# TheMTank/GridUniverse

Measured on AMD Instinct MI355X. Metric: env-steps/sec at N_envs on 32×32 grid, 1/2/4/8 MI355X; bit-exact vs CPU, higher is better.
Workload: dtype int32; 1 GPU; c3: 65536 envs per GPU on the 32x32 generator maze (random.seed(123); np.random.seed(123)), uniform device-RNG actions, auto-reset, 1000 env-steps per launch, int32 (obs,reward,done) rows; envs_per_gpu=65536, env_steps_per_launch=1000, global_envs=65536, parallelism=env-index shards, no data-path collective

## Files before the change

### griduniverse_amd/csrc/gu_internal.hpp

```cpp
#pragma once
#include <hip/hip_runtime.h>
#include <stdint.h>
#include <atomic>
#include <string>
#include <vector>

#include "../../include/gu.h"
#include "../../include/gu_diag.h"

#define GU_CELL_OPEN_MASK 0x0Fu
#define GU_CELL_TERM 0x10u
#define GU_CELL_TERM_BIT 4
#define GU_CELL_RPLUS 0x20u
#define GU_CELL_RMINUS 0x40u
#define GU_WIDE_STORE_PAD()                         \
    do {                                            \
        __builtin_amdgcn_sched_barrier(0);          \
        asm volatile("s_nop 1" ::: "memory");       \
        __builtin_amdgcn_sched_barrier(0);          \
    } while (0)
#define GU_ACTION_OK(raw) ((uint32_t)((int32_t)(raw) + 4) < 8u)
#define GU_CELL_WALL 0x80u

#define GU_MAX_LDS_CELLS 32767

#define GU_HOST_ERR_WORD 4
#define GU_HOST_COUNT_WORD 8

#define GU_STREAM_PAD_WORDS 4

struct GuPaceEntry {
    uint32_t period_q;
    uint32_t seq;
    uint64_t t_start;
    uint32_t unpaced;
    uint32_t phase;
    uint32_t left;
    uint32_t ema_paced;
    uint32_t ema_unpaced;
    uint32_t verdict;
    uint32_t waves;
    uint32_t elapsed;
    uint32_t ended_late;
    uint32_t max_behind;
    uint32_t report_steps;
    uint32_t groups;
    uint32_t dec_q;
    uint32_t block_left;
    uint32_t block_sum;
    uint32_t block_n;
    uint32_t last_mean;
    uint32_t up;
    uint32_t quiet;
    uint32_t reserved2[9];
};
static_assert(sizeof(GuPaceEntry) == 128, "GuPaceEntry is two cache lines' halves: 128 bytes");
#define GU_PACE_BLOCK 192u
#define GU_PACE_BLOCK_SKIP 64u
#define GU_PACE_NORMAL 0
#define GU_PACE_PROBE_OFF 1
#define GU_PACE_OFF 2
#define GU_PACE_PROBE_ON 3
#define GU_PACE_RING 64u
struct GuPaceArgs {
    GuPaceEntry *ring;
    uint64_t *slots;
    uint32_t seq;
    uint32_t period;
    uint32_t lo, hi;
    uint32_t groups;
    uint32_t report_at;
    uint32_t n_waves, slot_stride;
    uint16_t bar_num;
    uint16_t fixed;
    uint32_t gain_q;
    uint32_t dec_q;
    uint32_t probe_every;
    uint32_t adapt;
};

struct gu_engine {
    int device = -1;
    int n_cu = 256;
    int64_t lds_per_cu = 160 * 1024;
    bool gfx950 = true;
    int64_t opt[GU_OPT_COUNT];
    int64_t opt_x[GU_OPT_X_COUNT];
    hipStream_t stream = nullptr;
    hipEvent_t ev_begin = nullptr, ev_end = nullptr, ev_sync = nullptr;
    std::vector<hipEvent_t> ev_marks;
    size_t n_marks = 0;

    int64_t N = 0;
    int64_t env_id0 = 0;

    bool has_grid = false;
    int32_t W = 0, H = 0, S = 0;
    int32_t cell_bytes = 0;
    uint8_t *d_cell = nullptr;
    uint8_t *d_cell_raw = nullptr;
    uint8_t *d_kind = nullptr;
    uint64_t delta_lut = 0;
    int32_t *d_starts = nullptr;
    int32_t *d_nstarts = nullptr;
    int32_t n_starts = 0;
    int32_t start0 = 0;
    int32_t max_starts = 0;
    bool all_single_start = true;
    int32_t n_grids = 1;
    int64_t group = 0;

    int32_t *d_out3 = nullptr;
    uint32_t *d_episode = nullptr;
    int32_t *d_out3_alt = nullptr;
    uint32_t *d_episode_alt = nullptr;
    uint64_t *d_done_bits_alt = nullptr;
    uint32_t *d_nib = nullptr;
    bool nib_valid = false;
    uint32_t *d_tcount = nullptr;
    uint64_t steps_taken = 0;
    int64_t off_lo = 0, off_hi = 0;
    bool off_exact = true;
    uint64_t seed = 0;
    uint32_t seed_prefix = 0;

    int32_t *d_actions = nullptr;
    uint32_t *d_actions_packed = nullptr;
    int64_t actions_T = 0;
    int64_t actions_cap = 0;

    int32_t *d_traj = nullptr;
    int64_t traj_T = 0;
    int traj_kind = 0;
    int traj_written = 0;
    int32_t traj_candidates = 0;
    float traj_probe_ms_best = 0.0f, traj_probe_ms_worst = 0.0f;
    std::vector<float> traj_probe_ms;
    std::vector<uint64_t> traj_probe_addr;
    int32_t traj_kept = -1;
    float traj_search_ms = 0.0f;
    uint64_t traj_peak_bytes = 0;
    bool traj_registered = false;

    struct PaceKind {
        bool active = false;
        const void *buffer = nullptr;
        unsigned blocks = 0;
        int64_t T = 0;
        int row_bytes = 0;
        uint32_t seq = 0;
        uint32_t model = 0;
        uint32_t n_waves = 0;
    } pace[36];
    GuPaceEntry *d_pace_ring = nullptr;
    uint64_t *d_pace_slots = nullptr;
    int64_t pace_slot_stride = 0;
    hipEvent_t ev_cal[2] = {nullptr, nullptr};

    uint32_t *d_rows[2] = {nullptr, nullptr};
    int rows_shift[2] = {-1, -1};
    uint32_t *d_rows2[2] = {nullptr, nullptr};
    bool rows2_built[2] = {false, false};
    uint32_t *d_mrows[2] = {nullptr, nullptr}, *d_mrows1[2] = {nullptr, nullptr};
    int mrows_K[2] = {0, 0}, mrows_shift[2] = {-1, -1};
    uint32_t *d_prow = nullptr;

    int32_t *d_ret = nullptr;
    int32_t *d_episodes_fin = nullptr;
    bool stats_valid = false;

    uint64_t *d_done_bits = nullptr;
    bool entry_table_ok = false;
    bool done_bits_valid = false;

    void *d_scratch = nullptr;
    size_t scratch_bytes = 0;

    int32_t *h_pin = nullptr;
    double *h_tables = nullptr;
    size_t h_tables_bytes = 0;
    bool h_tables_valid = false;
    unsigned long long *h_ctl = nullptr;
    char *h_up = nullptr;
    uint32_t *h_seq = nullptr;
    uint32_t *d_blocks_done = nullptr;
    uint32_t seq = 0, seq_since_sync = 0;

    hipGraphExec_t graph_exec = nullptr;
    int64_t graph_t0 = -1, graph_T = -1;
    uint32_t graph_flags = 0;

    double *d_v[2] = {nullptr, nullptr};
    double *d_pi[2] = {nullptr, nullptr};
    uint4 *d_pi_thr = nullptr;
    int vi_cur = 0;
    bool has_vi = false;
    double *d_delta = nullptr;
    uint8_t *d_greedy = nullptr;
    bool greedy_valid = false;
    int32_t vi_xcd_members[8] = {0, 0, 0, 0, 0, 0, 0, 0};
    int vi_run_form = 0;
    void *d_vi_xcd_ctl = nullptr, *d_vi_xcd_work = nullptr;
    size_t vi_xcd_ctl_bytes = 0, vi_xcd_work_bytes = 0;
    uint32_t vi_xcd_epoch = 1;
    int64_t vi_xcd_torn = 0;
    int vi_dp_form = 0;

    double *d_q = nullptr;
    int8_t *d_td_next = nullptr;
    int32_t td_S = 0;
    bool td_carry = false;
    int32_t *d_nstep_sa = nullptr;
    int32_t *d_nstep_r = nullptr;
    int32_t *d_nstep_cnt = nullptr;
    int32_t nstep_key = 0;
    int32_t *d_lambda_w = nullptr;
    int32_t lambda_key = 0;
    double *d_ac_h = nullptr;
    double *d_ac_v = nullptr;
    int32_t ac_S = 0;
    int32_t *d_rf_buf = nullptr;
    int32_t *d_rf_cnt = nullptr;
    int32_t rf_cap = 0;
    int32_t rf_key = 0;
    double *d_is_c = nullptr;
    int32_t is_S = 0;
    double *d_is_R = nullptr;
    int64_t is_eps = -1;
    int32_t *d_is_buf = nullptr;
    int32_t *d_is_cnt = nullptr;
    int32_t is_cap = 0;
    int32_t is_key = 0;
    double *d_fa_w = nullptr;
    int32_t *d_fa_phi = nullptr;
    uint16_t *d_fa_phi16 = nullptr;
    size_t fa_phi16_bytes = 0;
    int8_t *d_fa_next = nullptr;
    int32_t fa_S = 0, fa_K = 0, fa_F = 0;
    bool fa_carry = false;
    uint64_t *d_dyna_model = nullptr;
    int32_t *d_dyna_list = nullptr;
    int32_t *d_dyna_count = nullptr;
    uint8_t *d_dyna_seen = nullptr;
    int32_t dyna_S = 0;
    bool dyna_exact = false;
    double *d_search_score = nullptr;
    int64_t *d_search_steps = nullptr;
    uint32_t *d_explore_n = nullptr;
    int32_t explore_S = 0;
    double *d_explore_tab = nullptr;
    int32_t explore_C = 0;
    uint8_t *d_mcts_pool = nullptr;
    int32_t *d_mcts_meta = nullptr;
    int32_t *d_mcts_nodes = nullptr;
    int64_t *d_mcts_steps = nullptr;
    int32_t mcts_P = 0;
    double *d_mcts_tab = nullptr;
    int32_t mcts_C = 0;

    int32_t trail_cap = 0;
    int32_t *d_trail = nullptr;
    int32_t *d_trail_len = nullptr, *d_trail_head = nullptr;
    uint8_t *d_trail_done = nullptr;
    uint32_t *d_trail_alpha = nullptr;

    void *comm = nullptr;
    int32_t nranks = 0, rank = 0;
    int32_t *d_gather = nullptr;

    int32_t *pos() const { return d_out3; }
    int32_t *reward() const { return d_out3 + N; }
    int32_t *done() const { return d_out3 + 2 * N; }
};

struct GridSel {
    int64_t group;
    int64_t grid_stride;
    const int32_t *n_starts;
    int32_t n_grids, max_starts;
    int32_t per_wave;
};

inline GridSel gu_grid_sel(const gu_engine *h)
{
    return GridSel{h->group, 2 * (int64_t)h->cell_bytes, h->d_nstarts, h->n_grids, h->max_starts, 0};
}

void gu_set_error(const char *fmt, ...);
int gu_fail(int code, const char *fmt, ...);

#define GU_HIP(expr)                                                                              \
    do {                                                                                          \
        hipError_t _e = (expr);                                                                   \
        if (_e != hipSuccess)                                                                     \
            return gu_fail(_e == hipErrorOutOfMemory ? GU_ERR_NOMEM : GU_ERR_HIP, "%s failed: %s", \
                           #expr, hipGetErrorString(_e));                                         \
    } while (0)

#define GU_REQUIRE(cond, code, ...) \
    do {                            \
        if (!(cond)) return gu_fail(code, __VA_ARGS__); \
    } while (0)

int gu_use_device(gu_engine *h);
int gu_ensure_scratch(gu_engine *h, size_t bytes);

#define GU_TRY(call)                                 \
    do {                                             \
        int _rc = (call);                            \
        if (_rc != GU_OK) return _rc;                \
    } while (0)

#define GU_ENTER(h) GU_TRY(gu_use_device(h))

#define GU_NEED_GRID(h) GU_REQUIRE((h)->has_grid, GU_ERR_STATE, "no grid set: call gu_set_grid first")

template <class... P>
static inline void gu_release(P *&...p)
{
    ((p ? (void)hipFree(p) : (void)0, p = nullptr), ...);
}

int64_t gu_opt(const gu_engine *h, int option);
int gu_debug();

template <typename K>
static inline void gu_allow_lds(K kern, std::atomic<uint64_t> &mask, int device, size_t bytes, size_t wanted)
{
    if (bytes <= 64 * 1024) return;
    const uint64_t bit = device < 64 ? (1ull << device) : 0;
    if (bit && (mask.load(std::memory_order_relaxed) & bit)) return;
    (void)hipFuncSetAttribute((const void *)kern, hipFuncAttributeMaxDynamicSharedMemorySize, (int)wanted);
    if (bit) mask.fetch_or(bit, std::memory_order_relaxed);
}

int gu_launch_reset(gu_engine *h, const uint8_t *d_mask, const int32_t *d_choice, bool only_done);
int gu_launch_step(gu_engine *h, const int32_t *d_actions_row, uint32_t flags, int32_t *host_obs = nullptr,
                   int32_t *host_reward = nullptr, int32_t *host_done = nullptr, uint32_t *host_seq = nullptr, uint32_t seq = 0,
                   uint32_t *host_err = nullptr);
int gu_launch_validate_actions(gu_engine *h, const int32_t *d_actions, int64_t count);
int gu_launch_pack_actions(gu_engine *h, int64_t T);
int gu_launch_rollout(gu_engine *h, int64_t T, int32_t policy, uint32_t flags);
int gu_launch_lookahead(gu_engine *h, int64_t n, const int32_t *d_states, const int32_t *d_actions, bool care,
                        int32_t *d_next, int32_t *d_reward, int32_t *d_done);
int gu_launch_done_compact(gu_engine *h);
int gu_launch_deinterleave(gu_engine *h, const int32_t *triples, int32_t *planes, int64_t count);
int gu_probe_trajectory_buffer(gu_engine *h, int32_t *buf, int64_t T, float *ms);
int gu_device_copy(gu_engine *h, void *dst, const void *src, size_t bytes);
#define GU_MAX_SEGMENTS 8
struct GuSegments {
    void *dst[GU_MAX_SEGMENTS];
    const void *src[GU_MAX_SEGMENTS];
    size_t words[GU_MAX_SEGMENTS];
    int n = 0;
    void add(void *d, const void *s, size_t bytes)
    {
        dst[n] = d, src[n] = s, words[n] = bytes / 4;
        ++n;
    }
};
int gu_device_segments(gu_engine *h, const GuSegments &s);
#define GU_CTL_WORDS (8 + 4096 + 20480)
#define GU_UP_BYTES (40 * 4096)
int gu_read_back(gu_engine *h, void *dst, const void *src, size_t bytes);

int gu_vi_alloc(gu_engine *h);
void gu_vi_free(gu_engine *h);
int gu_launch_greedy_table(gu_engine *h);

struct GuXcdPlan {
    int block = 0, K = 0, NB = 1;
    unsigned G = 0;
    uint32_t values = 0;
    size_t lds = 0, slots_bytes = 0, work_bytes = 0;
};
#define GU_VI_FALLBACK 1
bool gu_vi_xcd_plan(const gu_engine *h, bool agents, GuXcdPlan *plan);
void gu_vi_xcd_free(gu_engine *h);
int gu_vi_xcd_fused_run(gu_engine *h, const GuXcdPlan &xp, double gamma, int32_t iters, uint32_t flags, double *deltas);
int gu_vi_xcd_dp_run(gu_engine *h, double gamma, double threshold, bool use_threshold, bool greedy, int32_t max_rounds, int32_t *rounds_done,
                     double *deltas);

// ... 34 lines not shown
```

### griduniverse_amd/csrc/gu_rollout.hpp

```cpp
#pragma once
#include "gu_map.hpp"

#include <cstdlib>
#include <functional>
#include <type_traits>

__device__ __forceinline__ uint32_t gu_sample_action(uint32_t word, const uint4 q)
{
    return (uint32_t)(word >= q.x) + (uint32_t)(word >= q.y) + (uint32_t)(word >= q.z) - q.w;
}


#define GU_DPP_REDUCE(x, OP)                                                                                     \
    do {                                                                                                         \
        uint32_t o_;                                                                                             \
        o_ = (uint32_t)__builtin_amdgcn_update_dpp(0, (int)(x), 0x111, 0xF, 0xF, false), (x) = OP((x), o_);      \
        o_ = (uint32_t)__builtin_amdgcn_update_dpp(0, (int)(x), 0x112, 0xF, 0xF, false), (x) = OP((x), o_);      \
        o_ = (uint32_t)__builtin_amdgcn_update_dpp(0, (int)(x), 0x114, 0xF, 0xF, false), (x) = OP((x), o_);      \
        o_ = (uint32_t)__builtin_amdgcn_update_dpp(0, (int)(x), 0x118, 0xF, 0xF, false), (x) = OP((x), o_);      \
        o_ = (uint32_t)__builtin_amdgcn_update_dpp(0, (int)(x), 0x142, 0xA, 0xF, false), (x) = OP((x), o_);      \
        o_ = (uint32_t)__builtin_amdgcn_update_dpp(0, (int)(x), 0x143, 0xC, 0xF, false), (x) = OP((x), o_);      \
    } while (0)
#define GU_OP_ADD(a_, b_) ((a_) + (b_))
#define GU_OP_MAX(a_, b_) ((a_) > (b_) ? (a_) : (b_))

struct GuPacer {
    uint64_t due, t0;
    uint32_t ticks;
    uint32_t report_at;
    uint32_t n_steps;
    uint32_t p_q;
    uint64_t *slot;
    uint64_t w[16];
    uint32_t c_seq, c_phase, c_left, c_ema_p, c_ema_u, v_period_q, v_seq, v_unpaced, v_report_steps, v_groups;
    uint32_t c_dec_q, c_block_left, c_block_sum, c_block_n, c_last_mean, c_up, c_quiet;
    uint64_t v_t_start;
    bool first_wave;
    __device__ __forceinline__ void fetch(const GuPaceArgs &pa, bool on)
    {
        ticks = on ? pa.period : 0u;
        p_q = pa.period << 6;
        first_wave = false;
        if (on && pa.ring) {
            const GuPaceEntry *entry = pa.ring + (pa.seq & (GU_PACE_RING - 1u));
            const GuPaceEntry *prev = pa.ring + ((pa.seq - 1u) & (GU_PACE_RING - 1u));
            c_seq = entry->seq;
            const bool mine = c_seq == pa.seq;
            const uint32_t have = mine ? entry->period_q : 0u;
            const uint32_t unpaced = mine ? entry->unpaced : 0u;
            c_phase = entry->phase, c_left = entry->left, c_ema_p = entry->ema_paced, c_ema_u = entry->ema_unpaced;
            v_period_q = prev->period_q, v_seq = prev->seq, v_unpaced = prev->unpaced, v_t_start = prev->t_start;
            v_report_steps = prev->report_steps, v_groups = prev->groups;
            if (have && !pa.fixed) p_q = have;
            p_q = p_q < (pa.lo << 6) ? (pa.lo << 6) : p_q;
            p_q = p_q > (pa.hi << 6) ? (pa.hi << 6) : p_q;
            if (pa.fixed) p_q = pa.period << 6;
            ticks = (unpaced && !pa.fixed) ? 0u : (p_q + 32u) >> 6;
            c_quiet = (mine && !pa.fixed) ? entry->quiet : 0u;
            first_wave = blockIdx.x == 0 && __builtin_amdgcn_readfirstlane(threadIdx.x) < 64u;
            if (first_wave && !c_quiet) {
                c_dec_q = entry->dec_q, c_block_left = entry->block_left, c_block_sum = entry->block_sum, c_block_n = entry->block_n;
                c_last_mean = entry->last_mean, c_up = entry->up;
                const uint64_t *set = pa.slots + (size_t)((pa.seq - 1u) & 1u) * pa.slot_stride;
#pragma unroll
                for (uint32_t j = 0; j < 16u; ++j) {
                    const uint32_t i = j * 64u + threadIdx.x;
                    w[j] = i < pa.n_waves ? __builtin_nontemporal_load(set + i) : 0ull;
                }
            }
        }
    }
    __device__ __forceinline__ void start(const GuPaceArgs &pa, bool on)
    {
        slot = nullptr;
        n_steps = 0;
        report_at = 0;
        t0 = 0;
        if (on && pa.ring) {
            const uint64_t now = __builtin_amdgcn_s_memrealtime();
            due = t0 = now;
            if (c_quiet) {
                if (first_wave) decide_quiet(pa, now);
                return;
            }
            const uint32_t wave = __builtin_amdgcn_readfirstlane((blockIdx.x * blockDim.x + threadIdx.x) >> 6);
            slot = pa.slots + (size_t)(pa.seq & 1u) * pa.slot_stride + wave;
            report_at = pa.report_at;
            if (first_wave) decide(pa, now);
            return;
        }
        due = ticks ? __builtin_amdgcn_s_memrealtime() : 0ull;
    }
    __device__ __forceinline__ void decide_early(const GuPaceArgs &pa)
    {
        if (first_wave && !c_quiet) decide(pa, __builtin_amdgcn_s_memrealtime());
    }
    __device__ __forceinline__ void decide_quiet(const GuPaceArgs &pa, uint64_t now)
    {
        first_wave = false;
        if (threadIdx.x == 0) {
            GuPaceEntry *cur = pa.ring + (pa.seq & (GU_PACE_RING - 1u));
            GuPaceEntry *next = pa.ring + ((pa.seq + 1u) & (GU_PACE_RING - 1u));
            uint32_t ema_u = c_ema_u;
            const uint64_t gap = now - v_t_start;
            const uint32_t took = gap > 0x7FFFFFFFull ? 0x7FFFFFFFu : (uint32_t)gap;
            if (v_seq + 1u == pa.seq && v_unpaced && v_t_start && v_groups == pa.groups && (!ema_u || took < 2u * ema_u)) ema_u = ema_u ? (ema_u * 7u + took) >> 3 : took;
            cur->t_start = now, cur->groups = pa.groups, cur->report_steps = 0;
            const uint32_t left = c_left > 0u ? c_left - 1u : 0u;
            next->period_q = p_q, next->seq = pa.seq + 1u, next->t_start = 0, next->unpaced = 1u;
            next->phase = GU_PACE_OFF, next->left = left, next->ema_paced = c_ema_p, next->ema_unpaced = ema_u;
            next->verdict = 0, next->waves = 0, next->elapsed = 0, next->ended_late = 0, next->max_behind = 0, next->report_steps = 0, next->groups = 0;
            next->dec_q = pa.dec_q, next->block_left = GU_PACE_BLOCK, next->block_sum = 0, next->block_n = 0, next->last_mean = 0, next->up = 0;
            next->quiet = left > 1u ? 1u : 0u;
        }
    }
    __device__ __forceinline__ void decide(const GuPaceArgs &pa, uint64_t now)
    {
        first_wave = false;
        uint64_t *set = pa.slots + (size_t)((pa.seq - 1u) & 1u) * pa.slot_stride;
        GuPaceEntry *cur = pa.ring + (pa.seq & (GU_PACE_RING - 1u));
        GuPaceEntry *prev = pa.ring + ((pa.seq - 1u) & (GU_PACE_RING - 1u));
        const bool fresh = c_seq != pa.seq;
        const bool prev_ok = v_seq + 1u == pa.seq;
        const uint32_t prev_ticks = (prev_ok && !v_unpaced) ? (pa.fixed ? pa.period : (v_period_q + 32u) >> 6) : 0u;
        const uint32_t scheduled = (prev_ticks * ((v_report_steps + 15u) & ~15u)) >> 4;
        const bool same_length = v_groups == pa.groups;
        uint32_t counts = 0, most = 0, longest = 0;
        for (uint32_t base = 0; base < pa.n_waves; base += 64u * 16u) {
            if (base) {
#pragma unroll
                for (uint32_t j = 0; j < 16u; ++j) {
                    const uint32_t i = base + j * 64u + threadIdx.x;
                    w[j] = i < pa.n_waves ? __builtin_nontemporal_load(set + i) : 0ull;
                }
            }
#pragma unroll
            for (uint32_t j = 0; j < 16u; ++j) {
                const uint32_t i = base + j * 64u + threadIdx.x;
                if (i < pa.n_waves) set[i] = 0;
                const uint32_t reported = (uint32_t)(w[j] >> 63), elapsed = (uint32_t)w[j] & 0x7FFFFFFFu;
                const uint32_t behind = (prev_ticks && elapsed > scheduled) ? elapsed - scheduled : 0u;
                counts += (reported << 16) + ((reported && behind > 2u * prev_ticks) ? 1u : 0u);
                most = behind > most ? behind : most;
                longest = elapsed > longest ? elapsed : longest;
            }
        }
        GU_DPP_REDUCE(counts, GU_OP_ADD);
        GU_DPP_REDUCE(most, GU_OP_MAX);
        GU_DPP_REDUCE(longest, GU_OP_MAX);
        if (threadIdx.x == 63) {
            const uint32_t waves = counts >> 16, far = counts & 0xFFFFu;
            GuPaceEntry *next = pa.ring + ((pa.seq + 1u) & (GU_PACE_RING - 1u));
            uint32_t n_q = p_q, phase = GU_PACE_NORMAL, left = pa.probe_every ? (pa.probe_every < 128u ? pa.probe_every : 128u) : 0u, ema_p = 0, ema_u = 0;
            uint32_t dec_q = pa.dec_q, block_left = GU_PACE_BLOCK, block_sum = 0, block_n = 0, last_mean = 0, up = 0;
            if (!fresh) {
                phase = c_phase, left = c_left, ema_p = c_ema_p, ema_u = c_ema_u;
                dec_q = c_dec_q, block_left = c_block_left, block_sum = c_block_sum, block_n = c_block_n, last_mean = c_last_mean, up = c_up;
            } else {
                cur->unpaced = 0, cur->phase = phase, cur->left = left, cur->ema_paced = 0, cur->ema_unpaced = 0;
                cur->dec_q = dec_q, cur->block_left = block_left, cur->block_sum = 0, cur->block_n = 0, cur->last_mean = 0, cur->up = up;
            }
            cur->period_q = p_q, cur->seq = pa.seq, cur->t_start = now, cur->report_steps = pa.report_at, cur->groups = pa.groups;
            cur->verdict = 0, cur->waves = 0, cur->elapsed = 0, cur->ended_late = 0, cur->max_behind = 0;
            if (waves && prev_ok) {
                prev->verdict = (uint64_t)most * 256u > (uint64_t)prev_ticks * v_groups * pa.bar_num ? 2u : 1u;
                prev->waves = waves, prev->elapsed = longest, prev->ended_late = far, prev->max_behind = far ? most : 0u;
                const uint64_t gap = now - v_t_start;
                const uint32_t mean = v_unpaced ? ema_u : ema_p;
                const uint32_t took = gap > 0x7FFFFFFFull ? 0x7FFFFFFFu : (uint32_t)gap;
                const bool plausible = same_length && v_t_start && (!mean || took < 2u * mean);
                if (v_unpaced) {
                    if (plausible) ema_u = ema_u ? (ema_u + took) >> 1 : took;
                } else {
                    if (plausible) ema_p = ema_p ? (ema_p * 7u + took) >> 3 : took;
                    const uint32_t step_up = (uint32_t)(((uint64_t)pa.gain_q * far) / waves);
                    const uint32_t early = 512u / (8u + (pa.seq > 100000u ? 100000u : pa.seq));
                    const uint32_t dec = early > dec_q ? early : dec_q;
                    n_q += step_up;
                    n_q = n_q > dec ? n_q - dec : n_q;
                    if (phase == GU_PACE_NORMAL && !pa.fixed && pa.adapt) {
                        if (block_left <= GU_PACE_BLOCK - GU_PACE_BLOCK_SKIP && plausible) block_sum += took, ++block_n;
                        if (block_left) --block_left;
                        if (!block_left) {
                            const uint32_t mean = block_n ? block_sum / block_n : 0u;
                            if (mean && last_mean && mean > last_mean) up ^= 1u;
                            if (mean) last_mean = mean;
                            dec_q = up ? (dec_q * 4u + 2u) / 3u : (dec_q * 3u) / 4u;
                            dec_q = dec_q < 4u ? 4u : dec_q;
                            dec_q = dec_q > pa.gain_q / 8u ? pa.gain_q / 8u : dec_q;
                            block_left = GU_PACE_BLOCK, block_sum = 0, block_n = 0;
                        }
                    }
                }
            }
            n_q = n_q < (pa.lo << 6) ? (pa.lo << 6) : n_q;
            n_q = n_q > (pa.hi << 6) ? (pa.hi << 6) : n_q;
            if (pa.probe_every && !pa.fixed && left && --left == 0u) {
                const bool off_wins = ema_u && ema_p && (uint64_t)ema_u * 100u < (uint64_t)ema_p * 98u;
                if (phase != GU_PACE_NORMAL || off_wins) block_left = GU_PACE_BLOCK, block_sum = 0, block_n = 0, last_mean = 0;
                if (phase == GU_PACE_NORMAL) phase = GU_PACE_PROBE_OFF, left = 4u, ema_u = 0u;
                else if (phase == GU_PACE_OFF) phase = GU_PACE_PROBE_ON, left = 8u, ema_p = 0u;
                else if (off_wins) phase = GU_PACE_OFF, left = 2u * pa.probe_every;
                else phase = GU_PACE_NORMAL, left = pa.probe_every;
            }
            next->period_q = n_q, next->seq = pa.seq + 1u, next->t_start = 0;
            next->unpaced = (phase == GU_PACE_PROBE_OFF || phase == GU_PACE_OFF) ? 1u : 0u;
            next->phase = phase, next->left = left, next->ema_paced = ema_p, next->ema_unpaced = ema_u;
            next->dec_q = dec_q, next->block_left = block_left, next->block_sum = block_sum, next->block_n = block_n, next->last_mean = last_mean, next->up = up;
            next->quiet = (phase == GU_PACE_OFF && left > 1u) ? 1u : 0u;
            next->verdict = 0, next->waves = 0, next->elapsed = 0, next->ended_late = 0, next->max_behind = 0, next->report_steps = 0, next->groups = 0;
        }
    }
    __device__ __forceinline__ void report(uint64_t now)
    {
        if ((threadIdx.x & 63u) == 0u) {
            const uint64_t elapsed = now - t0;
            *slot = (1ull << 63) | (elapsed > 0x7FFFFFFFull ? 0x7FFFFFFFull : elapsed);
        }
        report_at = 0;
    }
    __device__ __forceinline__ bool idle() const { return ticks == 0u && slot == nullptr; }
    __device__ __forceinline__ void after(uint32_t steps)
    {
        if (ticks) {
            due += (ticks * steps) >> 4;
            const uint64_t now = __builtin_amdgcn_s_memrealtime();
            n_steps += steps;
            if (__builtin_expect(report_at != 0u && n_steps >= report_at, 0)) report(now);
            if ((int64_t)(now - due) < 0)
                for (uint32_t turn = 0; turn < 2u * ticks + 64u && (int64_t)(__builtin_amdgcn_s_memrealtime() - due) < 0; ++turn)
                    __builtin_amdgcn_s_sleep(1);
        } else if (slot) {
            n_steps += steps;
            if (__builtin_expect(report_at != 0u && n_steps >= report_at, 0)) report(__builtin_amdgcn_s_memrealtime());
        }
    }
    __device__ __forceinline__ void finish()
    {
        if (slot && report_at) report(__builtin_amdgcn_s_memrealtime());
    }
};

struct RolloutArgs {
    const uint8_t *cell;
    const uint8_t *greedy;
    const uint4 *pi_thr;
    int32_t S, pi_lds;
    int32_t cell_bytes, W;
    uint64_t lut;
    int32_t *pos, *reward, *done;
    uint32_t *episode;
    const uint32_t *tcount;
    const int32_t *starts;
    const uint32_t *actions;
    int32_t *tr_obs, *tr_reward, *tr_done;
    int32_t *ret, *episodes_fin;
    uint64_t *done_bits;
    uint32_t n_starts, seed_prefix, env_id0, steps_taken;
    uint32_t seed_prefix0, steps_hi;
    const uint32_t *nib;
    int32_t nib_dwords;
    uint64_t lut_p;
    int32_t straddle;
    int64_t N, T;
    GridSel gs;
    const uint32_t *rows;
    const uint32_t *rows2;
    int32_t row_shift;
    int32_t stream_lds_off;
    int32_t stream_lds_words;
    int32_t entry_table;
    int32_t half_waves;
    int32_t xcd_remap;
    GuPaceArgs pace;
};

__device__ __forceinline__ uint32_t gu_env_block(int32_t xcd_remap)
{
    const uint32_t b = blockIdx.x;
    return xcd_remap ? (b & 7u) * (gridDim.x >> 3) + (b >> 3) : b;
}

template <bool TAIL16 = false, class S16, class S1>
__device__ __forceinline__ void gu_stream_run(const char *pa, int64_t row, uint32_t e4, int64_t T, int64_t i0, S16 &&step16, S1 &&step1)
{
    const uint32_t row32 = (uint32_t)row;
    auto word_at = [&](int64_t k, uint32_t c) {
        return (uint32_t)__builtin_amdgcn_raw_buffer_load_b32(__builtin_amdgcn_make_buffer_rsrc((void *)(pa + k * row), 0, 0xFFFFFFFFu, 0x00020000), e4,
                                                              c * row32, 0);
    };
    int64_t i = i0, k = i0 >> 4;
    if (i & 15) {
        const uint32_t word = word_at(k, 0);
        for (; i < T && (i & 15); ++i) step1((word >> (2u * (uint32_t)(i & 15))) & 3u);
        ++k;
    }
    uint32_t w[4];
#pragma unroll
    for (uint32_t c = 0; c < 4; ++c) w[c] = word_at(k, c);
    for (const int64_t full = T >> 4; k + 4 <= full; k += 4, i += 64) {
#pragma unroll
        for (uint32_t c = 0; c < 4; ++c) {
            const uint32_t word = w[c];
            asm volatile("" ::"v"(word));
            w[c] = word_at(k + 4, c);
            step16(word);
        }
    }
    uint32_t q = 0;
    if (TAIL16) {
        for (; i + 16 <= T; i += 16, q += 16) {
            const uint32_t sel = q >> 4;
            step16(sel == 0 ? w[0] : sel == 1 ? w[1] : w[2]);
        }
    }
    for (; i < T; ++i, ++q) {
        const uint32_t sel = q >> 4, word = sel == 0 ? w[0] : sel == 1 ? w[1] : sel == 2 ? w[2] : w[3];
        step1((word >> (2u * (q & 15u))) & 3u);
    }
}

#ifndef GU_STORE_AUX
#define GU_STORE_AUX 18
#endif
#ifndef GU_STORE_AUX_PACKED
#define GU_STORE_AUX_PACKED 16
#endif
#define GU_MAX_BLOCK 1024
typedef uint32_t gu_v3u __attribute__((ext_vector_type(3)));
template <int POLICY, int AUTO, int TRAJ, bool STATS, int MAP>
__global__ void __launch_bounds__(GU_MAX_BLOCK) gu_rollout_kernel(const RolloutArgs a)
{
    constexpr bool LDS = MAP == 1 || MAP == 3;
    extern __shared__ __attribute__((aligned(16))) uint8_t smem[];
    GuPacer pacer;
    pacer.fetch(a.pace, TRAJ == 1 || TRAJ == 3);
    const int64_t e64 = (int64_t)gu_env_block(a.xcd_remap) * blockDim.x + threadIdx.x;
    const bool live = e64 < a.N;
    const uint32_t e = (uint32_t)e64;
    int32_t s = 0, r = 0;
    uint32_t d = 0, ep = 0, tcount0 = 0;
    if (live) {
        s = a.pos[e];
        r = a.reward[e];
        d = (uint32_t)a.done[e];
        ep = a.episode[e];
        tcount0 = a.tcount[e];
    }
    CellMap m = gu_stage_map<LDS>(a.cell, a.cell_bytes, smem, a.gs, MAP == 3 ? 1 : 2);
    const uint32_t nib_region = MAP == 5 ? (threadIdx.x >> 6) * (uint32_t)a.nib_dwords * 256u : 0u;
    if (MAP == 5) {
        const size_t wave = ((size_t)blockIdx.x * blockDim.x + threadIdx.x) >> 6;
        const uint4 *src = reinterpret_cast<const uint4 *>(a.nib + wave * (size_t)a.nib_dwords * 64u);
        uint4 *dst = reinterpret_cast<uint4 *>(smem + nib_region);
        if (wave * 64u < (size_t)a.N)
            for (int32_t i = threadIdx.x & 63; i < a.nib_dwords * 16; i += 64) dst[i] = src[i];
        __syncthreads();
    }
    const uint8_t *greedy = a.greedy;
    if (MAP == 1 && POLICY == GU_POLICY_GREEDY) {
        uint8_t *dst = smem + 2 * a.cell_bytes;
        for (int32_t i = threadIdx.x * 16; i < a.cell_bytes; i += blockDim.x * 16)
            *reinterpret_cast<uint4 *>(dst + i) = *reinterpret_cast<const uint4 *>(a.greedy + i);
        __syncthreads();
        greedy = dst;
    }
    const bool thr_in_lds = MAP == 1 && POLICY == GU_POLICY_SAMPLE && a.pi_lds;
    uint4 *thr_lds = reinterpret_cast<uint4 *>(smem + 2 * a.cell_bytes);
    if (thr_in_lds) {
        for (int32_t i = threadIdx.x; i < a.S; i += blockDim.x) thr_lds[i] = a.pi_thr[i];
        __syncthreads();
    }
    if (!live) return;
    LaneGrid lg = gu_lane_grid<LDS>(a.gs, a.starts, a.n_starts, e, m);

    const uint32_t t_lane = tcount0 + a.steps_taken;
    const uint32_t prefix = gu_rng_prefix(a.seed_prefix, a.env_id0 + e);
    const uint32_t prefix0 = AUTO == 2 ? gu_rng_prefix(a.seed_prefix0, a.env_id0 + e) : prefix;
    const uint32_t epoch0 = (uint32_t)((uint64_t)((int64_t)(((uint64_t)a.steps_hi << 32) | a.steps_taken) + (int64_t)(int32_t)tcount0) >> 32);
    auto prefix_at = [&](uint32_t t) {
        return gu_rng_prefix(gu_rng_seed_prefix_epoch(a.seed_prefix0, epoch0 + (t < t_lane ? 1u : 0u)), a.env_id0 + e);
    };
    constexpr uint32_t TERM5 = 0x20u, TERM5_BIT = 5u;
    auto flags5 = [](uint32_t b) { return (((b >> 5) & 3u) << 3) | (((b >> GU_CELL_TERM_BIT) & 1u) << TERM5_BIT) | ((b >> 7) << 6); };
    uint32_t flags = MAP == 5 ? flags5(m.f[s]) : m.f[s];
    int32_t ret = 0, fin = 0;
    const int32_t W = a.W;
    const uint64_t lut = a.lut;
    const int32_t start0 = lg.starts[0];
    const uint32_t start0_flags = MAP == 5 ? flags5(m.f[start0]) : m.f[start0];
    auto padded = [&](int32_t c) { return (int32_t)(((uint32_t)(c + c / W + W + 2) << 5) + nib_region); };
    int32_t sq = MAP == 5 ? padded(s) : 0;
    const int32_t start0_q = MAP == 5 ? padded(start0) : 0;
    typedef __attribute__((address_space(3))) const uint32_t *lds_word_ptr;
    const uint32_t lane4 = (threadIdx.x & 63u) << 2;
    auto word_at = [&](int32_t cq) { return *(lds_word_ptr)(uintptr_t)(((uint32_t)cq & 0xFFFFFF00u) | lane4); };
    auto four_of = [](uint32_t word, int32_t cq) { return __builtin_amdgcn_ubfe(word, (uint32_t)cq >> 3, 4); };
    auto four_at = [&](int32_t cq) { return four_of(word_at(cq), cq); };
    auto cell5 = [&](int32_t cq) { return four_at(cq) << 3; };
    auto move5 = [&](uint32_t act, int32_t delta, auto &&in_the_shadow) {
        int32_t cand = s + delta;
        asm volatile("" : "+v"(cand));
        const int32_t candq = sq + gu_delta<true>(act, a.lut_p, 0);
        const uint32_t word = word_at(candq);
        in_the_shadow();
        const uint32_t four = four_of(word, candq);
        const bool go = ((flags & TERM5) | four) < 8u;
        s = go ? cand : s;
        sq = go ? candq : sq;
        flags = go ? four << 3 : flags;
    };
    char *po = (char *)a.tr_obs, *pr = (char *)a.tr_reward, *pd = (char *)a.tr_done;
    const char *pa = (const char *)a.actions;
    const uint32_t e4 = e * 4u;
    const int64_t row = a.N * 4;
    const uint32_t row32 = (uint32_t)row;
    const int64_t trow = TRAJ == 3 ? a.N * 12 : row;
    const uint32_t trow32 = (uint32_t)trow;
    const uint32_t te = TRAJ == 3 ? e * 12u : e4;
    __amdgpu_buffer_rsrc_t ro = __builtin_amdgcn_make_buffer_rsrc(po, 0, 0xFFFFFFFFu, 0x00020000);
    __amdgpu_buffer_rsrc_t rr = __builtin_amdgcn_make_buffer_rsrc(pr, 0, 0xFFFFFFFFu, 0x00020000);
    __amdgpu_buffer_rsrc_t rd = __builtin_amdgcn_make_buffer_rsrc(pd, 0, 0xFFFFFFFFu, 0x00020000);
    auto emit = [&](int32_t s_, int32_t r_, uint32_t d_, uint32_t soff) {
        if (TRAJ == 1) {
            __builtin_amdgcn_raw_buffer_store_b32(s_, ro, e4, soff, GU_STORE_AUX);
            __builtin_amdgcn_raw_buffer_store_b32(r_, rr, e4, soff, GU_STORE_AUX);
            __builtin_amdgcn_raw_buffer_store_b32((int32_t)d_, rd, e4, soff, GU_STORE_AUX);
        } else if (TRAJ == 2) {
            __builtin_amdgcn_raw_buffer_store_b32((int32_t)((uint32_t)s_ | (((uint32_t)r_ & 0xFFu) << 16) | (d_ << 24)), ro, e4, soff, GU_STORE_AUX_PACKED);
        } else if (TRAJ == 3) {
            const gu_v3u triple = {(uint32_t)s_, (uint32_t)r_, d_};
            __builtin_amdgcn_raw_buffer_store_b96(triple, ro, te, soff, GU_STORE_AUX);
            GU_WIDE_STORE_PAD();
        }
    };
    bool held = false;
    int32_t held_s = 0, held_r = 0;
    uint32_t held_d = 0, held_soff = 0;
    auto release = [&]() {
        if (MAP == 5 && TRAJ && held) emit(held_s, held_r, held_d, held_soff);
        held = false;
    };
    auto rebase = [&](int64_t rows) {
        release();
        po += rows * trow;
        ro = __builtin_amdgcn_make_buffer_rsrc(po, 0, 0xFFFFFFFFu, 0x00020000);
        if (TRAJ == 1) {
            pr += rows * trow;
            pd += rows * trow;
            rr = __builtin_amdgcn_make_buffer_rsrc(pr, 0, 0xFFFFFFFFu, 0x00020000);
            rd = __builtin_amdgcn_make_buffer_rsrc(pd, 0, 0xFFFFFFFFu, 0x00020000);
        }
    };

    if (AUTO == 1 && MAP != 5) flags = (flags & ~GU_CELL_TERM) | (d << GU_CELL_TERM_BIT);

    auto step = [&](uint32_t act, uint32_t soff) {
        const int32_t delta = gu_delta<MAP != 0>(act, lut, W);
        if (AUTO == 1) {
            const bool was_done = MAP == 5 ? d != 0u : (flags & GU_CELL_TERM) != 0u;
            ep += was_done;
            s = was_done ? start0 : s;
            flags = was_done ? start0_flags : flags;
            if (MAP == 5) sq = was_done ? start0_q : sq;
        } else if (AUTO == 2) {
            if (d) {
                s = lg.starts[gu_rng_start_index(prefix0, ep, lg.n_starts)];
                ++ep;
                if (MAP == 5) sq = padded(s);
                flags = MAP == 5 ? cell5(sq) : m.f[s];
            }
        }
        if (MAP == 5) {
            move5(act, delta, [&]() {
                if (TRAJ && held) {
                    __builtin_amdgcn_sched_barrier(0);
                    emit(held_s, held_r, held_d, held_soff);
                    __builtin_amdgcn_sched_barrier(0);
                }
            });
        } else {
            s = gu_move(s, flags, act, delta);
            flags = m.f[s];
        }
        r = MAP == 5 ? __builtin_amdgcn_sbfe((int32_t)0xF6F60AFFu, flags, 8) : (MAP >= 2) ? gu_reward_packed(flags) : (int32_t)m.r[s];
        d = __builtin_amdgcn_ubfe(flags, MAP == 5 ? TERM5_BIT : GU_CELL_TERM_BIT, 1);
        if (STATS) {
            ret += r;
            fin += (int32_t)d;
        }
        if (MAP == 5 && TRAJ) held = true, held_s = s, held_r = r, held_d = d, held_soff = soff;
        else emit(s, r, d, soff);
    };
    auto step1 = [&](uint32_t act) {
        step(act, 0);
        if (TRAJ) rebase(1);
    };

    pacer.start(a.pace, TRAJ == 1 || TRAJ == 3);
    if (POLICY == GU_POLICY_UNIFORM && a.straddle) {
        uint32_t t = t_lane;
#pragma nounroll
        for (int64_t i = 0; i < a.T; ++i, ++t) step1((gu_rng_word(prefix_at(t), GU_RNG_STREAM_ACTION, t >> 4) >> (2u * (t & 15u))) & 3u);
    } else if (POLICY == GU_POLICY_UNIFORM) {
        const uint32_t t_first = __builtin_amdgcn_readfirstlane(t_lane);
        if (__all(t_lane == t_first)) {
            uint32_t t = t_first;
            int64_t i = 0;
            if (t & 15u) {
                const uint32_t word = gu_rng_word(prefix, GU_RNG_STREAM_ACTION, t >> 4);
                for (; i < a.T && (t & 7u); ++i, ++t) step1((word >> (2u * (t & 15u))) & 3u);
                if ((t & 15u) == 8u && i + 8 <= a.T) {
// ... 297 lines not shown
```

Baseline: 598.8 billion env-steps/s.

## Add startup search phases to adaptive pacing controller and factor rule into shared header

Moves the wave-pacing control law into a host/device header and extends it with a startup state machine. The machine gathers background lateness statistics, seeds the decay rate, then tries mid/up/down decay settings over short blocks and keeps the best before normal adaptation. It also caps per-step increases and speeds travel during the skipped part of a block. The aim is to reach a good pacing period in fewer launches than the slow block-by-block search, at the cost of more controller state and new tuning constants.

Measured after the change: 598.5 billion env-steps/s (median of 2 runs). No clear change (-0.0%).

```diff
diff --git a/griduniverse_amd/csrc/gu_internal.hpp b/griduniverse_amd/csrc/gu_internal.hpp
--- a/griduniverse_amd/csrc/gu_internal.hpp
+++ b/griduniverse_amd/csrc/gu_internal.hpp
@@ -29,6 +29,7 @@
 
 #define GU_STREAM_PAD_WORDS 4
 
+#include "gu_pace_rule.hpp"
 struct GuPaceEntry {
     uint32_t period_q;
     uint32_t seq;
@@ -52,32 +53,15 @@
     uint32_t last_mean;
     uint32_t up;
     uint32_t quiet;
-    uint32_t reserved2[9];
+    uint32_t start;
+    uint32_t bg_far, bg_waves;
+    uint32_t bg_period_q;
+    uint32_t dec_mid;
+    uint32_t mean_mid, mean_up;
+    uint32_t reserved2[2];
 };
 static_assert(sizeof(GuPaceEntry) == 128, "GuPaceEntry is two cache lines' halves: 128 bytes");
-#define GU_PACE_BLOCK 192u
-#define GU_PACE_BLOCK_SKIP 64u
-#define GU_PACE_NORMAL 0
-#define GU_PACE_PROBE_OFF 1
-#define GU_PACE_OFF 2
-#define GU_PACE_PROBE_ON 3
 #define GU_PACE_RING 64u
-struct GuPaceArgs {
-    GuPaceEntry *ring;
-    uint64_t *slots;
-    uint32_t seq;
-    uint32_t period;
-    uint32_t lo, hi;
-    uint32_t groups;
-    uint32_t report_at;
-    uint32_t n_waves, slot_stride;
-    uint16_t bar_num;
-    uint16_t fixed;
-    uint32_t gain_q;
-    uint32_t dec_q;
-    uint32_t probe_every;
-    uint32_t adapt;
-};
 
 struct gu_engine {
     int device = -1;
diff --git a/griduniverse_amd/csrc/gu_pace_rule.hpp b/griduniverse_amd/csrc/gu_pace_rule.hpp
--- /dev/null
+++ b/griduniverse_amd/csrc/gu_pace_rule.hpp
@@ -0,0 +1,167 @@
+#pragma once
+#include <cstdint>
+
+#if defined(__HIPCC__)
+#define GU_HD __host__ __device__
+#else
+#define GU_HD
+#endif
+
+struct GuPaceEntry;
+
+#define GU_PACE_BLOCK 192u
+#define GU_PACE_BLOCK_SKIP 64u
+#define GU_PACE_NORMAL 0
+#define GU_PACE_PROBE_OFF 1
+#define GU_PACE_OFF 2
+#define GU_PACE_PROBE_ON 3
+#define GU_PACE_START_DONE 0u
+#define GU_PACE_START_BG 1u
+#define GU_PACE_START_MID 2u
+#define GU_PACE_START_UP 3u
+#define GU_PACE_START_DOWN 4u
+#define GU_PACE_START_HOLD 5u
+#define GU_PACE_BG_FIRST 4u
+#define GU_PACE_BG_LAST 9u
+#define GU_PACE_TRAVEL_DEC 48u
+
+struct GuPaceArgs {
+    GuPaceEntry *ring;
+    uint64_t *slots;
+    uint32_t seq;
+    uint32_t period;
+    uint32_t lo, hi;
+    uint32_t groups;
+    uint32_t report_at;
+    uint32_t n_waves, slot_stride;
+    uint16_t bar_num;
+    uint16_t fixed;
+    uint32_t gain_q;
+    uint32_t dec_q;
+    uint32_t probe_every;
+    uint32_t adapt;
+};
+
+struct GuPaceLoop {
+    uint32_t period_q;
+    uint32_t phase, left, ema_paced, ema_unpaced;
+    uint32_t dec_q, block_left, block_sum, block_n, last_mean, up;
+    uint32_t start, bg_far, bg_waves, bg_period_q, dec_mid, mean_mid, mean_up;
+};
+
+struct GuPaceReport {
+    uint32_t waves, far;
+    uint32_t most, longest;
+    uint32_t took;
+    uint32_t plausible;
+    uint32_t unpaced;
+};
+
+GU_HD inline uint32_t gu_pace_block_len(uint32_t start)
+{
+    return start == GU_PACE_START_DONE ? GU_PACE_BLOCK : start == GU_PACE_START_MID ? 86u : 32u;
+}
+GU_HD inline uint32_t gu_pace_block_skip(uint32_t start)
+{
+    return start == GU_PACE_START_DONE ? GU_PACE_BLOCK_SKIP : start == GU_PACE_START_MID ? 62u : 8u;
+}
+GU_HD inline uint32_t gu_pace_aim_clamp(uint32_t dec_q, const GuPaceArgs &pa)
+{
+    dec_q = dec_q < 4u ? 4u : dec_q;
+    return dec_q > pa.gain_q / 8u ? pa.gain_q / 8u : dec_q;
+}
+
+GU_HD inline GuPaceLoop gu_pace_first(uint32_t p_q, const GuPaceArgs &pa)
+{
+    GuPaceLoop s = {};
+    s.period_q = p_q;
+    s.phase = GU_PACE_NORMAL;
+    s.left = pa.probe_every ? (pa.probe_every < 128u ? pa.probe_every : 128u) : 0u;
+    s.dec_q = pa.dec_q;
+    s.block_left = GU_PACE_BLOCK;
+    s.start = (pa.adapt && !pa.fixed) ? GU_PACE_START_BG : GU_PACE_START_DONE;
+    return s;
+}
+
+GU_HD inline GuPaceLoop gu_pace_rule(GuPaceLoop s, const GuPaceReport &r, const GuPaceArgs &pa)
+{
+    uint32_t n_q = s.period_q;
+    if (s.phase == GU_PACE_OFF || s.phase == GU_PACE_PROBE_ON || pa.fixed || !pa.adapt) s.start = GU_PACE_START_DONE;
+    if (r.waves) {
+        const uint32_t mean = r.unpaced ? s.ema_unpaced : s.ema_paced;
+        const bool plausible = r.plausible && (!mean || r.took < 2u * mean);
+        if (r.unpaced) {
+            if (plausible) s.ema_unpaced = s.ema_unpaced ? (s.ema_unpaced + r.took) >> 1 : r.took;
+        } else {
+            if (plausible) s.ema_paced = s.ema_paced ? (s.ema_paced * 7u + r.took) >> 3 : r.took;
+            uint32_t gain_q = pa.gain_q, dec_q = s.dec_q;
+            const bool travels = s.phase == GU_PACE_NORMAL && s.start >= GU_PACE_START_MID && s.block_left > gu_pace_block_len(s.start) - gu_pace_block_skip(s.start);
+            if (travels && dec_q && dec_q < GU_PACE_TRAVEL_DEC) {
+                const uint32_t k = GU_PACE_TRAVEL_DEC / dec_q < 6u ? GU_PACE_TRAVEL_DEC / dec_q : 6u;
+                gain_q *= k, dec_q *= k;
+            }
+            uint32_t step_up = (uint32_t)(((uint64_t)gain_q * r.far) / r.waves);
+            step_up = step_up > pa.gain_q ? pa.gain_q : step_up;
+            const uint32_t early = 512u / (8u + (pa.seq > 100000u ? 100000u : pa.seq));
+            const uint32_t dec = early > dec_q ? early : dec_q;
+            n_q += step_up;
+            n_q = n_q > dec ? n_q - dec : n_q;
+            if (s.phase == GU_PACE_NORMAL && !pa.fixed && pa.adapt) {
+                if (s.start == GU_PACE_START_BG) {
+                    if (pa.seq >= GU_PACE_BG_FIRST) s.bg_far += r.far, s.bg_waves += r.waves, s.bg_period_q = s.period_q;
+                    if (pa.seq >= GU_PACE_BG_LAST) {
+                        uint32_t seed = s.bg_waves ? (uint32_t)((4ull * pa.gain_q * s.bg_far) / s.bg_waves) : 0u;
+                        seed = seed > (s.dec_q * 3u + 1u) / 2u ? (s.dec_q * 3u + 1u) / 2u : seed;
+                        s.dec_q = gu_pace_aim_clamp(seed > s.dec_q ? seed : s.dec_q, pa);
+                        s.start = GU_PACE_START_MID;
+                        s.block_left = gu_pace_block_len(s.start), s.block_sum = 0, s.block_n = 0;
+                    }
+                } else {
+                    if (s.start == GU_PACE_START_MID && s.block_left == gu_pace_block_len(s.start) - gu_pace_block_skip(s.start) && s.period_q + (6u << 6) > s.bg_period_q)
+                        s.dec_q = gu_pace_aim_clamp(pa.dec_q, pa), s.bg_far = 0, s.bg_waves = 0;
+                    const bool counts = plausible && (s.start == GU_PACE_START_DONE || r.took < s.ema_paced + s.ema_paced / 4u);
+                    if (s.block_left <= gu_pace_block_len(s.start) - gu_pace_block_skip(s.start) && counts) s.block_sum += r.took, ++s.block_n;
+                    if (s.block_left) --s.block_left;
+                    if (!s.block_left) {
+                        const uint32_t mean = s.block_n ? s.block_sum / s.block_n : 0u;
+                        if (s.start == GU_PACE_START_DONE) {
+                            if (mean && s.last_mean && mean > s.last_mean) s.up ^= 1u;
+                            if (mean) s.last_mean = mean;
+                            s.dec_q = gu_pace_aim_clamp(s.up ? (s.dec_q * 4u + 2u) / 3u : (s.dec_q * 3u) / 4u, pa);
+                        } else if (s.start == GU_PACE_START_MID) {
+                            s.dec_mid = s.dec_q, s.mean_mid = mean;
+                            s.dec_q = gu_pace_aim_clamp((s.dec_mid * 3u + 1u) / 2u, pa), s.start = GU_PACE_START_UP;
+                        } else if (s.start == GU_PACE_START_UP) {
+                            s.mean_up = mean;
+                            const uint32_t floor_q = s.bg_waves ? (uint32_t)((2ull * pa.gain_q * s.bg_far) / s.bg_waves) : 0u;
+                            s.dec_q = gu_pace_aim_clamp((s.dec_mid * 2u) / 3u > floor_q ? (s.dec_mid * 2u) / 3u : floor_q, pa), s.start = GU_PACE_START_DOWN;
+                        } else if (s.start == GU_PACE_START_DOWN) {
+                            uint32_t best = s.mean_mid;
+                            const uint32_t dec_down = s.dec_q, bar = best - best / 128u;
+                            s.dec_q = s.dec_mid, s.up = 0u;
+                            if (s.mean_up && (!best || s.mean_up < best - best / 48u)) best = s.mean_up, s.dec_q = gu_pace_aim_clamp((s.dec_mid * 3u + 1u) / 2u, pa), s.up = 1u;
+                            if (mean && (!best || mean < (s.up ? best : bar))) best = mean, s.dec_q = dec_down, s.up = 0u;
+                            s.last_mean = best, s.start = GU_PACE_START_HOLD;
+                        } else {
+                            if (mean) s.last_mean = mean;
+                            s.start = GU_PACE_START_DONE;
+                        }
+                        s.block_left = gu_pace_block_len(s.start), s.block_sum = 0, s.block_n = 0;
+                    }
+                }
+            }
+        }
+    }
+    n_q = n_q < (pa.lo << 6) ? (pa.lo << 6) : n_q;
+    n_q = n_q > (pa.hi << 6) ? (pa.hi << 6) : n_q;
+    if (pa.probe_every && !pa.fixed && s.left && --s.left == 0u) {
+        const bool off_wins = s.ema_unpaced && s.ema_paced && (uint64_t)s.ema_unpaced * 100u < (uint64_t)s.ema_paced * 98u;
+        if (s.phase != GU_PACE_NORMAL || off_wins) s.block_left = gu_pace_block_len(s.start), s.block_sum = 0, s.block_n = 0, s.last_mean = 0;
+        if (s.phase == GU_PACE_NORMAL) s.phase = GU_PACE_PROBE_OFF, s.left = 4u, s.ema_unpaced = 0u;
+        else if (s.phase == GU_PACE_OFF) s.phase = GU_PACE_PROBE_ON, s.left = 8u, s.ema_paced = 0u;
+        else if (off_wins) s.phase = GU_PACE_OFF, s.left = 2u * pa.probe_every;
+        else s.phase = GU_PACE_NORMAL, s.left = pa.probe_every;
+    }
+    s.period_q = n_q;
+    return s;
+}
diff --git a/griduniverse_amd/csrc/gu_rollout.hpp b/griduniverse_amd/csrc/gu_rollout.hpp
--- a/griduniverse_amd/csrc/gu_rollout.hpp
+++ b/griduniverse_amd/csrc/gu_rollout.hpp
@@ -34,6 +34,7 @@
     uint64_t w[16];
     uint32_t c_seq, c_phase, c_left, c_ema_p, c_ema_u, v_period_q, v_seq, v_unpaced, v_report_steps, v_groups;
     uint32_t c_dec_q, c_block_left, c_block_sum, c_block_n, c_last_mean, c_up, c_quiet;
+    uint32_t c_start, c_bg_far, c_bg_waves, c_bg_period_q, c_dec_mid, c_mean_mid, c_mean_up;
     uint64_t v_t_start;
     bool first_wave;
     __device__ __forceinline__ void fetch(const GuPaceArgs &pa, bool on)
@@ -61,6 +62,7 @@
             if (first_wave && !c_quiet) {
                 c_dec_q = entry->dec_q, c_block_left = entry->block_left, c_block_sum = entry->block_sum, c_block_n = entry->block_n;
                 c_last_mean = entry->last_mean, c_up = entry->up;
+                c_start = entry->start, c_bg_far = entry->bg_far, c_bg_waves = entry->bg_waves, c_bg_period_q = entry->bg_period_q, c_dec_mid = entry->dec_mid, c_mean_mid = entry->mean_mid, c_mean_up = entry->mean_up;
                 const uint64_t *set = pa.slots + (size_t)((pa.seq - 1u) & 1u) * pa.slot_stride;
 #pragma unroll
                 for (uint32_t j = 0; j < 16u; ++j) {
@@ -149,65 +151,36 @@
         GU_DPP_REDUCE(most, GU_OP_MAX);
         GU_DPP_REDUCE(longest, GU_OP_MAX);
         if (threadIdx.x == 63) {
-            const uint32_t waves = counts >> 16, far = counts & 0xFFFFu;
             GuPaceEntry *next = pa.ring + ((pa.seq + 1u) & (GU_PACE_RING - 1u));
-            uint32_t n_q = p_q, phase = GU_PACE_NORMAL, left = pa.probe_every ? (pa.probe_every < 128u ? pa.probe_every : 128u) : 0u, ema_p = 0, ema_u = 0;
-            uint32_t dec_q = pa.dec_q, block_left = GU_PACE_BLOCK, block_sum = 0, block_n = 0, last_mean = 0, up = 0;
+            GuPaceLoop s = gu_pace_first(p_q, pa);
             if (!fresh) {
-                phase = c_phase, left = c_left, ema_p = c_ema_p, ema_u = c_ema_u;
-                dec_q = c_dec_q, block_left = c_block_left, block_sum = c_block_sum, block_n = c_block_n, last_mean = c_last_mean, up = c_up;
+                s.phase = c_phase, s.left = c_left, s.ema_paced = c_ema_p, s.ema_unpaced = c_ema_u;
+                s.dec_q = c_dec_q, s.block_left = c_block_left, s.block_sum = c_block_sum, s.block_n = c_block_n, s.last_mean = c_last_mean, s.up = c_up;
+                s.start = c_start, s.bg_far = c_bg_far, s.bg_waves = c_bg_waves, s.bg_period_q = c_bg_period_q, s.dec_mid = c_dec_mid, s.mean_mid = c_mean_mid, s.mean_up = c_mean_up;
             } else {
-                cur->unpaced = 0, cur->phase = phase, cur->left = left, cur->ema_paced = 0, cur->ema_unpaced = 0;
-                cur->dec_q = dec_q, cur->block_left = block_left, cur->block_sum = 0, cur->block_n = 0, cur->last_mean = 0, cur->up = up;
+                cur->unpaced = 0, cur->phase = s.phase, cur->left = s.left, cur->ema_paced = 0, cur->ema_unpaced = 0;
+                cur->dec_q = s.dec_q, cur->block_left = s.block_left, cur->block_sum = 0, cur->block_n = 0, cur->last_mean = 0, cur->up = 0;
+                cur->start = s.start, cur->bg_far = 0, cur->bg_waves = 0, cur->bg_period_q = 0, cur->dec_mid = 0, cur->mean_mid = 0, cur->mean_up = 0;
             }
             cur->period_q = p_q, cur->seq = pa.seq, cur->t_start = now, cur->report_steps = pa.report_at, cur->groups = pa.groups;
             cur->verdict = 0, cur->waves = 0, cur->elapsed = 0, cur->ended_late = 0, cur->max_behind = 0;
-            if (waves && prev_ok) {
+            GuPaceReport r = {};
+            if ((counts >> 16) && prev_ok) {
+                r.waves = counts >> 16, r.far = counts & 0xFFFFu, r.most = most, r.longest = longest;
                 prev->verdict = (uint64_t)most * 256u > (uint64_t)prev_ticks * v_groups * pa.bar_num ? 2u : 1u;
-                prev->waves = waves, prev->elapsed = longest, prev->ended_late = far, prev->max_behind = far ? most : 0u;
+                prev->waves = r.waves, prev->elapsed = longest, prev->ended_late = r.far, prev->max_behind = r.far ? most : 0u;
                 const uint64_t gap = now - v_t_start;
-                const uint32_t mean = v_unpaced ? ema_u : ema_p;
-                const uint32_t took = gap > 0x7FFFFFFFull ? 0x7FFFFFFFu : (uint32_t)gap;
-                const bool plausible = same_length && v_t_start && (!mean || took < 2u * mean);
-                if (v_unpaced) {
-                    if (plausible) ema_u = ema_u ? (ema_u + took) >> 1 : took;
-                } else {
-                    if (plausible) ema_p = ema_p ? (ema_p * 7u + took) >> 3 : took;
-                    const uint32_t step_up = (uint32_t)(((uint64_t)pa.gain_q * far) / waves);
-                    const uint32_t early = 512u / (8u + (pa.seq > 100000u ? 100000u : pa.seq));
-                    const uint32_t dec = early > dec_q ? early : dec_q;
-                    n_q += step_up;
-                    n_q = n_q > dec ? n_q - dec : n_q;
-                    if (phase == GU_PACE_NORMAL && !pa.fixed && pa.adapt) {
-                        if (block_left <= GU_PACE_BLOCK - GU_PACE_BLOCK_SKIP && plausible) block_sum += took, ++block_n;
-                        if (block_left) --block_left;
-                        if (!block_left) {
-                            const uint32_t mean = block_n ? block_sum / block_n : 0u;
-                            if (mean && last_mean && mean > last_mean) up ^= 1u;
-                            if (mean) last_mean = mean;
-                            dec_q = up ? (dec_q * 4u + 2u) / 3u : (dec_q * 3u) / 4u;
-                            dec_q = dec_q < 4u ? 4u : dec_q;
-                            dec_q = dec_q > pa.gain_q / 8u ? pa.gain_q / 8u : dec_q;
-                            block_left = GU_PACE_BLOCK, block_sum = 0, block_n = 0;
-                        }
-                    }
-                }
-            }
-            n_q = n_q < (pa.lo << 6) ? (pa.lo << 6) : n_q;
-            n_q = n_q > (pa.hi << 6) ? (pa.hi << 6) : n_q;
-            if (pa.probe_every && !pa.fixed && left && --left == 0u) {
-                const bool off_wins = ema_u && ema_p && (uint64_t)ema_u * 100u < (uint64_t)ema_p * 98u;
-                if (phase != GU_PACE_NORMAL || off_wins) block_left = GU_PACE_BLOCK, block_sum = 0, block_n = 0, last_mean = 0;
-                if (phase == GU_PACE_NORMAL) phase = GU_PACE_PROBE_OFF, left = 4u, ema_u = 0u;
-                else if (phase == GU_PACE_OFF) phase = GU_PACE_PROBE_ON, left = 8u, ema_p = 0u;
-                else if (off_wins) phase = GU_PACE_OFF, left = 2u * pa.probe_every;
-                else phase = GU_PACE_NORMAL, left = pa.probe_every;
-            }
-            next->period_q = n_q, next->seq = pa.seq + 1u, next->t_start = 0;
-            next->unpaced = (phase == GU_PACE_PROBE_OFF || phase == GU_PACE_OFF) ? 1u : 0u;
-            next->phase = phase, next->left = left, next->ema_paced = ema_p, next->ema_unpaced = ema_u;
-            next->dec_q = dec_q, next->block_left = block_left, next->block_sum = block_sum, next->block_n = block_n, next->last_mean = last_mean, next->up = up;
-            next->quiet = (phase == GU_PACE_OFF && left > 1u) ? 1u : 0u;
+                r.took = gap > 0x7FFFFFFFull ? 0x7FFFFFFFu : (uint32_t)gap;
+                r.plausible = (same_length && v_t_start) ? 1u : 0u;
+                r.unpaced = v_unpaced;
+            }
+            s = gu_pace_rule(s, r, pa);
+            next->period_q = s.period_q, next->seq = pa.seq + 1u, next->t_start = 0;
+            next->unpaced = (s.phase == GU_PACE_PROBE_OFF || s.phase == GU_PACE_OFF) ? 1u : 0u;
+            next->phase = s.phase, next->left = s.left, next->ema_paced = s.ema_paced, next->ema_unpaced = s.ema_unpaced;
+            next->dec_q = s.dec_q, next->block_left = s.block_left, next->block_sum = s.block_sum, next->block_n = s.block_n, next->last_mean = s.last_mean, next->up = s.up;
+            next->start = s.start, next->bg_far = s.bg_far, next->bg_waves = s.bg_waves, next->bg_period_q = s.bg_period_q, next->dec_mid = s.dec_mid, next->mean_mid = s.mean_mid, next->mean_up = s.mean_up;
+            next->quiet = (s.phase == GU_PACE_OFF && s.left > 1u) ? 1u : 0u;
             next->verdict = 0, next->waves = 0, next->elapsed = 0, next->ended_late = 0, next->max_behind = 0, next->report_steps = 0, next->groups = 0;
         }
     }
```
